# drdh/Homophily-MARL

Measured on AMD Instinct MI355X. Metric: agent_steps_per_sec, higher is better.
Workload: dtype fp32

## Files before the change

### homophily_marl_amd/abi.py

```python
import ctypes as C
import os

ABI_VERSION = 10
MAX_AGENTS = 10
MAX_CELLS = 1024
MAX_SITES = 256

ENV_CLEANUP, ENV_HARVEST = 0, 1
RNG_TAPE, RNG_COUNTER = 0, 1
OBS_F32, OBS_BF16, OBS_U8, OBS_CODE = 0, 1, 2, 3
COLOR_SIMPLIFIED, COLOR_FULL = 0, 1
CODE_CLASS, CODE_CHANNEL_MASK = 0, 1
INPUT_LAST_ACTION, INPUT_AGENT_ID, INPUT_REWARD, INPUT_INC_REWARD, INPUT_DISTANCE, INPUT_AGENT_POS = 1, 2, 4, 8, 16, 32
INPUT_OTHERS_LAST_ACTION = 64
INPUT_GATHER_ONEHOT = 0x100
PREV_RECORD_BYTES = 16
INPUT_EXPLICIT = 0x80000000
STREAM_UNIFORM, STREAM_MOVE, STREAM_WASTE, STREAM_SPAWN_ROT = 0, 1, 2, 3

SSD_OK, SSD_ERR_INVALID, SSD_ERR_DEVICE, SSD_ERR_NOMEM, SSD_ERR_UNSUPPORTED = 0, -1, -2, -3, -4


class SsdConfig(C.Structure):
    _fields_ = [
# ... 135 lines not shown
                ("recv_inc", C.c_void_p), ("recv_inc_out", C.c_void_p), ("avail_bits", C.c_uint32),
                ("others_rows", C.c_void_p), ("prev_record", C.c_void_p), ("prev_record_out", C.c_void_p), ("onehot_rows", C.c_void_p)]


class SsdPolicyHeadParams(C.Structure):
    _fields_ = [("fc1_w", C.c_void_p), ("fc1_b", C.c_void_p), ("w_i", C.c_void_p * 3), ("w_h", C.c_void_p * 3), ("b_i", C.c_void_p * 3),
                ("b_h", C.c_void_p * 3), ("fc2_w", C.c_void_p), ("fc2_b", C.c_void_p), ("fc2_v_w", C.c_void_p), ("fc2_v_b", C.c_void_p),
                ("n_agents", C.c_int32), ("fc1_in", C.c_int32), ("fc2_in", C.c_int32), ("fc2_out", C.c_int32),
                ("input_flags", C.c_uint32), ("n_actions", C.c_int32), ("others_rows", C.c_void_p), ("onehot_rows", C.c_void_p)]


class SsdPolicyEncodeArgs(C.Structure):
    _fields_ = [("codes", C.c_void_p), ("code_bytes", C.c_int64), ("env_stride", C.c_int64), ("slot_stride", C.c_int64),
                ("agent_stride", C.c_int64), ("slot_t", C.c_void_p),
                ("rows", C.c_int32), ("view_edge", C.c_int32), ("n_agents", C.c_int32), ("agent_major", C.c_int32), ("precision", C.c_int32),
                ("conv_frags", C.c_void_p), ("lin_frags", C.c_void_p), ("conv_b", C.c_void_p), ("lin_b", C.c_void_p),
                ("out", C.c_void_p), ("out_stride", C.c_int32), ("part", C.c_void_p), ("slot_t_copy", C.c_void_p), ("counter_inc", C.c_void_p),
                ("alphabet", C.c_int32), ("act", C.c_void_p), ("slot_add", C.c_int32), ("layout", C.c_int32)]


class SsdTdLossArgs(C.Structure):
    _fields_ = [("batch", C.c_int32), ("t_slots", C.c_int32), ("n_agents", C.c_int32), ("n_actions", C.c_int32), ("sim_horizon", C.c_int32),
                ("double_q", C.c_int32),
                ("gamma_env", C.c_float), ("gamma_inc", C.c_float), ("reward_scale", C.c_float), ("incentive_ratio", C.c_float),
                ("incentive_cost", C.c_float), ("incentive", C.c_float), ("seq_len", C.c_float), ("sim_threshold", C.c_float),
                ("sim_loss_weight", C.c_float),
                ("q_env", C.c_void_p), ("q_inc", C.c_void_p), ("tq_env", C.c_void_p), ("tq_inc", C.c_void_p),
                ("actions", C.c_void_p), ("actions_inc", C.c_void_p), ("avail", C.c_void_p), ("reward", C.c_void_p), ("clean_num", C.c_void_p),
                ("terminated", C.c_void_p), ("filled", C.c_void_p), ("dens", C.c_void_p),
                ("dq_env", C.c_void_p), ("dq_inc", C.c_void_p), ("partials", C.c_void_p), ("consider_others_inc", C.c_int32)]


TD_LOSS_PARTIALS = 16
POLICY_HEAD_FRAGS, POLICY_HEAD_TAIL_FLOATS = 58, 464 + 64


POLICY_TAIL_PIECES = 3


def onehot_rows(n_agents, n_actions, flags):
    return 1 + 2 * n_actions + (n_agents * n_actions if flags & INPUT_OTHERS_LAST_ACTION else 0)


def policy_image_bytes(precision):
    return (56 * precision + 8) * 1024


def policy_tail_piece(precision):
    return 56 * precision + 2 * precision


def policy_frag_piece(precision, F, term):
    if F < 8:
        c, ot = F & 1, F >> 1
    elif F < 56:
        G = (F - 8) % 24
        c, ot = (8 if F >= 32 else 2) + 2 * (G >> 3) + (G & 1), (G & 7) >> 1
    else:
        return 56 * precision + 2 * term + (F - 56)
    return 4 * precision * c + 4 * term + ot


def policy_head_plan(n_env, n_agents, fused_with_encoder=False):
    lib = load_library()
    a, b, c = C.c_int32(0), C.c_int32(0), C.c_int32(0)
    check(lib, lib.ssd_policy_head_plan(n_env, n_agents, int(bool(fused_with_encoder)), C.byref(a), C.byref(b), C.byref(c)))
    return a.value, b.value, c.value


ENCODE_EDGE_MIN, ENCODE_EDGE_MAX, ENCODE_BANDS_MAX = 3, 63, 6


def encode_edge_supported(V):
    return ENCODE_EDGE_MIN <= V <= ENCODE_EDGE_MAX and V % 2 == 1


def encode_band_rows(V):
    O = V - 2
    nb = 1 if O <= 13 else min(ENCODE_BANDS_MAX, (O + 9) // 10)
    return (O + nb - 1) // nb


def encode_bands(V):
    return (V - 2 + encode_band_rows(V) - 1) // encode_band_rows(V)


ENCODE_LAYOUT_TOEPLITZ, ENCODE_LAYOUT_LUT = 0, 1
ENCODE_LUT_TABLE_BYTES = 3 * 64 * 6 * 4


def encode_lut_ksteps(V):
    O, R, nb = V - 2, encode_band_rows(V), encode_bands(V)
    return (nb - 1) * ((R * O + 3) // 4) + ((O - (nb - 1) * R) * O + 3) // 4


def encode_frag_bytes(V, precision, layout=ENCODE_LAYOUT_TOEPLITZ):
    if layout == ENCODE_LAYOUT_LUT:
        return ENCODE_LUT_TABLE_BYTES, encode_lut_ksteps(V) * 2 * precision * 1024
    units = 29 * 2 * 3 if V == 31 else 13 * 3
    return precision * 9 * 1024, units * 2 * precision * 1024


def code_agent_stride(V):
    return (V * V + 15) & ~15


HIP_SIGNATURES["ssd_policy_head_env"] = (C.c_int, [C.POINTER(SsdPolicyHead), C.c_void_p])
HIP_SIGNATURES["ssd_policy_head_inc"] = (C.c_int, [C.POINTER(SsdPolicyHead), C.c_void_p])
HIP_SIGNATURES["ssd_gru_seq_fwd"] = (C.c_int, [C.c_void_p] * 6 + [C.c_int32] * 3 + [C.c_void_p])
HIP_SIGNATURES["ssd_gru_seq_bwd"] = (C.c_int, [C.c_void_p] * 9 + [C.c_int32] * 3 + [C.c_void_p])
# ... 100 lines not shown
```

### homophily_marl_amd/csrc/ssd_policy_mfma.hip

```cpp
#include "ssd_policy_common.h"

namespace ssd {
#define SSD_GLOBAL __attribute__((address_space(1)))


using f32x4 = __attribute__((ext_vector_type(4))) float;
using u32x4 = __attribute__((ext_vector_type(4))) uint32_t;
using u32x2 = __attribute__((ext_vector_type(2))) uint32_t;
using h8 = __attribute__((ext_vector_type(8))) _Float16;
using b8 = __attribute__((ext_vector_type(8))) __bf16;

template <int PREC>
__device__ __forceinline__ f32x4 mma(u32x4 a, u32x4 b, f32x4 c) {
    if constexpr (PREC == 2) return __builtin_amdgcn_mfma_f32_16x16x32_f16(__builtin_bit_cast(h8, a), __builtin_bit_cast(h8, b), c, 0, 0, 0);
    else return __builtin_amdgcn_mfma_f32_16x16x32_bf16(__builtin_bit_cast(b8, a), __builtin_bit_cast(b8, b), c, 0, 0, 0);
}

template <int PREC>
__device__ __forceinline__ void split8(const float (&v)[8], u32x4& hi, u32x4& lo) {
    if constexpr (PREC == 2) {
        h8 h, l;
#pragma unroll
        for (int j = 0; j < 8; ++j) { h[j] = (_Float16)v[j]; l[j] = (_Float16)(v[j] - (float)h[j]); }
        hi = __builtin_bit_cast(u32x4, h); lo = __builtin_bit_cast(u32x4, l);
// ... 34 lines not shown
    for (int p = 0; p < 3; ++p) {
        const f32x2 x = x3[p];
        const f32x2 y = x * c;
        float m0, m1, l0, l1;
        asm("v_max_f32 %0, %1, %2" : "=v"(m0) : "v"(x.x), "v"(y.x));
        asm("v_max_f32 %0, %1, %2" : "=v"(m1) : "v"(x.y), "v"(y.y));
        uint32_t h, l;
        asm("v_cvt_pk_f16_f32 %0, %1, %2" : "=v"(h) : "v"(m0), "v"(m1));
        asm("v_fma_mix_f32 %0, %1, -1.0, %2 op_sel:[0,0,0] op_sel_hi:[1,0,0]" : "=v"(l0) : "v"(h), "v"(m0));
        asm("v_fma_mix_f32 %0, %1, -1.0, %2 op_sel:[1,0,0] op_sel_hi:[1,0,0]" : "=v"(l1) : "v"(h), "v"(m1));
        asm("v_cvt_pk_f16_f32 %0, %1, %2" : "=v"(l) : "v"(l0), "v"(l1));
        hi[p] = h; lo[p] = l;
    }
    hi[3] = 0u; lo[3] = 0u;
#else
    (void)x3; hi = u32x4{0u, 0u, 0u, 0u}; lo = hi;
#endif
}

template <int PREC> __device__ __forceinline__ void store_term(uint8_t* dst, float v, size_t term_stride, int32_t* err) {
    if constexpr (PREC == 2) {
        if (!(fabsf(v) <= F16_MAX) && err) atomicOr(err, ERR_F16_RANGE);
        const _Float16 h = (_Float16)v, l = (_Float16)(v - (float)h);
        *reinterpret_cast<_Float16*>(dst) = h; *reinterpret_cast<_Float16*>(dst + term_stride) = l;
    } else {
        *reinterpret_cast<__bf16*>(dst) = (__bf16)v;
    }
}

#ifdef SSD_STAMPS
static unsigned long long* g_policy_stamps = nullptr;
void set_policy_stamps(unsigned long long* buf) { g_policy_stamps = buf; }
#define PSTAMP_DECL unsigned long long* stamps;
#define PSTAMP_SET(k) (k).stamps = g_policy_stamps
#define PSTAMP_AT(i, v) do { if (a.stamps && lane == 0) a.stamps[((size_t)(blockIdx.y * gridDim.x + blockIdx.x) * (blockDim.x >> 6) + wave) * 16 + (i)] = (v); } while (0)
#define PSTAMP(i) PSTAMP_AT(i, __builtin_amdgcn_s_memtime())
#define PSTAMP_REAL(i) PSTAMP_AT(i, __builtin_amdgcn_s_memrealtime())
#define PSTAMP_DRAINED(i) do { asm volatile("s_waitcnt vmcnt(0) lgkmcnt(0)" ::: "memory"); PSTAMP(i); } while (0)
#else
#define PSTAMP_DECL
#define PSTAMP_SET(k)
#define PSTAMP(i)
#define PSTAMP_REAL(i)
#define PSTAMP_DRAINED(i)
#endif

constexpr float HEAD_WSCALE = 64.f, HEAD_XSCALE = 16.f;
constexpr float ENC_CSCALE = 256.f, ENC_LSCALE = 256.f;

constexpr int HF_WI = 8, HF_WH = 32, HF_FC2 = 56, HF_TOT = SSD_POLICY_HEAD_FRAGS;
constexpr int HT_B1 = 0, HT_BI = 64, HT_BH = 256, HT_B2 = 448, HT_W2O = 464, HT_TOT = SSD_POLICY_HEAD_TAIL_FLOATS;
constexpr int SCRATCH = 16 * 16;
constexpr int HEAD_STEPS = 14;
template <int PREC> constexpr int stream_chunks() { return HEAD_STEPS * 4 * PREC / 8; }
template <int PREC> constexpr int step_piece(int c, int t, int ot) { return 4 * PREC * c + 4 * t + ot; }
template <int PREC> constexpr int res_piece() { return stream_chunks<PREC>() * 8; }
template <int PREC> constexpr int fc2_piece(int t, int s2) { return res_piece<PREC>() + 2 * t + s2; }
template <int PREC> constexpr int tail_piece() { return res_piece<PREC>() + 2 * PREC; }
static_assert(res_piece<2>() + 8 == SSD_POLICY_IMAGE_PIECES(2) && res_piece<1>() + 8 == SSD_POLICY_IMAGE_PIECES(1), "image = stream chunks + resident chunk");
static_assert(tail_piece<2>() + SSD_POLICY_TAIL_PIECES <= SSD_POLICY_IMAGE_PIECES(2) && tail_piece<1>() + SSD_POLICY_TAIL_PIECES <= SSD_POLICY_IMAGE_PIECES(1), "tail fits");
constexpr int cmin(int a, int b) { return a < b ? a : b; }
constexpr int cmax(int a, int b) { return a > b ? a : b; }

__device__ __forceinline__ void dma_piece(const uint8_t* gsrc_lane, uint32_t lds_dst) {
#if defined(__HIP_DEVICE_COMPILE__)
    uint32_t keep;
    asm volatile("s_mov_b32 %0, m0\n\ts_mov_b32 m0, %2\n\ts_nop 0\n\tglobal_load_lds_dwordx4 %1, off\n\ts_mov_b32 m0, %0"
                 : "=&s"(keep) : "v"(gsrc_lane), "s"(lds_dst) : "memory");
#else
    (void)gsrc_lane; (void)lds_dst;
#endif
}
template <int N> __device__ __forceinline__ void wait_vm() {
#if defined(__HIP_DEVICE_COMPILE__)
    asm volatile("s_waitcnt vmcnt(%0)" : : "n"(N) : "memory");
#endif
}
using lds_u32 = __attribute__((address_space(3))) uint32_t;
constexpr int STREAM_AHEAD = 6;
constexpr int head_lds_bytes(int waves, int prec) { return SSD_POLICY_IMAGE_BYTES(prec) + waves * SCRATCH * 4 + 16; }
template <int PREC>
__device__ __forceinline__ void stream_image(const uint8_t* src_lane, uint32_t lds_dst, volatile lds_u32* landed) {
    constexpr int NK = stream_chunks<PREC>(), NC = NK + 1;
    auto issue = [&](int k) {
        const int j = k == 0 ? NK : k - 1;
#pragma unroll
        for (int pc = 0; pc < 8; ++pc) dma_piece(src_lane + (size_t)j * 8192 + pc * 1024, lds_dst + (uint32_t)j * 8192u + (uint32_t)pc * 1024u);
    };
#pragma unroll
    for (int k = 0; k < cmin(STREAM_AHEAD + 1, NC); ++k) issue(k);
#pragma unroll
    for (int k = 0; k < NC; ++k) {
        if (k + STREAM_AHEAD < NC) wait_vm<8 * STREAM_AHEAD>();
        else if (k == NC - 1) wait_vm<0>();
        else if (k == NC - 2) wait_vm<8>();
        else if (k == NC - 3) wait_vm<16>();
        else if (k == NC - 4) wait_vm<24>();
        else if (k == NC - 5) wait_vm<32>();
        else wait_vm<40>();
        *landed = (uint32_t)k;
        if (k + STREAM_AHEAD + 1 < NC) issue(k + STREAM_AHEAD + 1);
    }
}
template <int PREC, int C> __device__ __forceinline__ void chunk_ready(volatile const lds_u32* landed, uint32_t& seen) {
    constexpr int first_piece = step_piece<PREC>(C, 0, 0), j = first_piece >> 3;
    if constexpr ((first_piece & 7) == 0) {
// ... 296 lines not shown
        (void)lane;
        PSTAMP(0);
        PSTAMP_REAL(14);
        if (!LOOP && wave < WAVES) {
            const int bia0 = block - (block / a.bpa) * a.bpa, tile00 = wave * a.bpa + bia0;
            if (tile00 < ((a.N + 15) >> 4)) load_tile_rows<INC, PRE_SMALL>(a, tile00, block / a.bpa, lane, in_rows);
        }
        if (!LOOP) {
            if (!INC) asm volatile("" :: "s"(a.N), "s"(a.n), "s"(a.bpa), "s"(a.h), "s"(a.inputs), "s"(a.weights), "s"(a.eps), "s"(a.step), "s"(a.t_index),
                                         "s"(a.prev_actions), "s"(a.prev_reward), "s"(a.recv), "s"(a.prev_inc), "s"(a.pos), "s"(a.orient), "s"(a.feat_part),
                                         "s"(a.lin_b), "s"(a.feat_bands), "s"(a.avail_bits), "s"(a.pos_scale));
            else asm volatile("" :: "s"(a.N), "s"(a.n), "s"(a.bpa), "s"(a.h), "s"(a.inputs), "s"(a.weights), "s"(a.eps), "s"(a.step), "s"(a.t_index),
                                    "s"(a.actions), "s"(a.pos_pre), "s"(a.orient_pre), "s"(a.reward), "s"(a.clean), "s"(a.den), "s"(a.ep_ret), "s"(a.term),
                                    "s"(a.inp), "s"(a.pos_scale));
        }
        if (wave == WAVES) *landed = 0u;
        __builtin_amdgcn_s_barrier();
        if (wave == WAVES) {
            const int agent = block / a.bpa;
            stream_image<PREC>(a.weights + (size_t)agent * IMAGE_BYTES + lane * 16, (uint32_t)(uintptr_t)lds_raw, landed);
            return;
        }
    }
    auto pass = [&](const HeadK& a, const int lane, const int tile) {
    const int agent = block / a.bpa;
    const int m = lane & 15, q = lane >> 4;
    const int N = a.N, n = a.n;
    const int tiles = (N + 15) >> 4;
    TileIn<INC> in;
    if constexpr (!LOOP) in = in_rows;
    if (!INC) PSTAMP_DRAINED(8);
    if (!INC) PSTAMP(9);
    float eps = *(const float SSD_GLOBAL*)a.eps;
    int64_t step64 = *(const int64_t SSD_GLOBAL*)a.step;
    long slot_t = a.t_index ? (long)*(const int64_t SSD_GLOBAL*)a.t_index : 0;
    if (tile < tiles) {
        if constexpr (LOOP) load_tile<INC, false>(a, tile, agent, lane, in);
        else if (!INC && a.feat_part) { load_tile<INC, false, PRE_SMALL>(a, tile, agent, lane, in); }
        else load_tile<INC, true, PRE_SMALL>(a, tile, agent, lane, in);
    }
    u32x4 prec = {0xFFFFFFFFu, 0xFFFFFFFFu, 0xFFFFFFFFu, 0xFFFFFFFFu};
    if constexpr (GEN >= 2) {
        if (tile < tiles) {
            auto rec = cold_ptr<const uint8_t>(COLD_BASE, gather_slots<INC>() + 8);
            const int b0 = tile * 16 + m, bc0 = b0 < N ? b0 : N - 1;
            prec = *(const u32x4 SSD_GLOBAL*)(rec + (size_t)bc0 * 16);
        }
    }
    f32x4 gsum[4];
    if (!INC) PSTAMP(10);
    uint32_t step = 0;
    bool file = false;
    const uint32_t avail_bits = INC ? 0xFFFFFFFFu : ((a.avail_bits >> 31) ? (a.avail_bits & 0x7FFFFFFFu) : avail_to_bits(a.avail, A));
    if (!INC) PSTAMP_DRAINED(11);
    u32x4 bh[2], bl[2];
    auto range_check = [&](float amax) {
        if (!(amax * XS <= F16_MAX)) {
            auto nerr = COLD(int32_t, numeric_err);
            if (nerr) atomicOr((int32_t*)nerr, ERR_F16_RANGE);
        }
    };
    f32x4 xk[4];
    auto prepare = [&](int tl) {
        const int b = tl * 16 + m;
        const bool valid = b < N;
        const int bc = valid ? b : N - 1;
        f32x4 (&x)[4] = xk;
        if (!INC) {
            x[0] = in.x[0]; x[1] = in.x[1];
            if (a.feat_part) {
#pragma unroll
                for (int ct = 0; ct < 2; ++ct) {
#pragma unroll
                    for (int r = 0; r < 4; ++r) x[ct][r] = leaky(x[ct][r]);
                }
            }
            int o_act = 0, o_id = A, o_r = A + n, o_i = A + n + 1, o_dist = TAIL_ABSENT, o_pos = A + n + 2;
            if (GEN) {
                const uint64_t lay = COLD_U64(tail_layout);
                o_act = (int8_t)lay; o_id = (int8_t)(lay >> 8); o_r = (int8_t)(lay >> 16); o_i = (int8_t)(lay >> 24);
                o_dist = (int8_t)(lay >> 32); o_pos = (int8_t)(lay >> 40);
            }
            const float px = in.p0 / a.pos_scale, py = in.p1 / a.pos_scale;
            int recv = 0;
#pragma unroll
            for (int k = 0; k < 3; ++k) {
                const int g = q + 4 * k;
                const int on = (g < n && g != agent) ? 1 : 0;
                recv += on * ((in.inc[k] == 1) - (in.inc[k] == 2));
            }
            recv += __builtin_popcount(in.rv & 0x01010101u) - __builtin_popcount(in.rv & 0x02020202u);
            recv += __shfl_xor(recv, 16);
            recv += __shfl_xor(recv, 32);
            const float sg_r = (float)((in.pr > 0.f) - (in.pr < 0.f)), sg_i = (float)((recv > 0) - (recv < 0));
            const int c_pa = o_act + in.pa, c_id = o_id + agent;
#pragma unroll
            for (int ct = 2; ct < 4; ++ct) {
#pragma unroll
                for (int r = 0; r < 4; ++r) {
                    const int j = 16 * ct + 4 * q + r - 32;
                    float v = (j == c_pa || j == c_id) ? 1.f : 0.f;
                    v = j == o_r ? sg_r : v;
                    v = j == o_i ? sg_i : v;
                    v = j == o_pos ? px : v;
                    v = j == o_pos + 1 ? py : v;
                    x[ct][r] = v;
                }
// ... 75 lines not shown
#pragma unroll
                        for (int ot = 0; ot < 4; ++ot) part[k][ot] = *(const f32x4 SSD_GLOBAL*)((const uint8_t SSD_GLOBAL*)orows + (size_t)((row * 64u + 16u * ot + 4u * (uint32_t)q) * 4u));
                    }
#pragma unroll
                    for (int k = 0; k < 3; ++k) {
                        if (g0 + k >= SSD_MAX_AGENTS) continue;
#pragma unroll
                        for (int ot = 0; ot < 4; ++ot)
#pragma unroll
                            for (int r = 0; r < 4; ++r) {
                                const float v = part[k][ot][r];
                                gsum[ot][r] += __builtin_bit_cast(float, __builtin_bit_cast(uint32_t, v) & keep[k]);
                            }
                    }
                }
            }
        }
    };
    auto file_inputs = [&](int tl) {
        if (INC) return;
        const int b = tl * 16 + m;
        if (b >= N) return;
        float* in_row = a.inputs + ((size_t)agent * N + b) * 64;
#pragma unroll
        for (int ct = 0; ct < 4; ++ct)
            if (ct >= 2 || a.feat_part) stg128(in_row, (size_t)((16 * ct + 4 * q) * 4), xk[ct]);
        if (q == 0) {
            const size_t er = (size_t)b * n + agent;
            ColdA ca; ColdC cc;
            cold_blocks(COLD_BASE, ca, nullptr, &cc);
            const float o0 = a.orient ? in.o0 : 0.f, o1 = a.orient ? in.o1 : 0.f;
            if (ca.pos_copy) {
                ca.pos_copy[er * 2] = in.p0; ca.pos_copy[er * 2 + 1] = in.p1; ca.orient_copy[er * 2] = o0; ca.orient_copy[er * 2 + 1] = o1;
            }
            if (cc.d_pos && file) {
                const size_t sr = (((size_t)b * a.slots + slot_t) * n + agent) * 2;
                cc.d_pos[sr] = in.p0; cc.d_pos[sr + 1] = in.p1; cc.d_orient[sr] = o0; cc.d_orient[sr + 1] = o1;
            }
        }
    };
    auto hand_counters = [&]() {
      if (block == 0 && tid == 0) {
        if (INC) {
            auto next_t = COLD(int64_t, next_t); auto next_step = COLD(int64_t, next_step);
            if (next_t) *next_t = slot_t + 1;
            if (next_step) *next_step = step64 + 1;
        } else {
            auto t_copy = COLD(int64_t, t_copy); auto step_copy = COLD(int64_t, step_copy);
            if (t_copy) *t_copy = slot_t;
            if (step_copy) *step_copy = step64;
        }
      }
    };
    PSTAMP(12);
    step = (uint32_t)step64;
    file = slot_t < (long)a.slots;
    if (tile < tiles) prepare(tile);
    PSTAMP(13);
    PSTAMP(1);
    const uint8_t* img = lds_raw;
    const float* tail = reinterpret_cast<const float*>(img + (size_t)tail_piece<PREC>() * 1024);
    float* scratch = reinterpret_cast<float*>(lds_raw + IMAGE_BYTES) + wave * SCRATCH;
    auto run_tile = [&]() {
        if (PREC == 2) range_check(amax_tiles<4>(0.f, xk));
        const int b = tile * 16 + m;
        const bool valid = b < N;
        const int bc = valid ? b : N - 1;
        const size_t arow = (size_t)agent * N + bc;
        if (first) PSTAMP(2);
        f32x4 x1[4];
#pragma unroll
        for (int ot = 0; ot < 4; ++ot) x1[ot] = f32x4{0.f, 0.f, 0.f, 0.f};
        Frag4<PREC> fa, fb;
#define SSD_LOAD_STEP(c_, f_) do { chunk_ready<PREC, c_>(landed, seen); frag4_load<PREC>(img, c_, lane, f_); } while (0)
        SSD_LOAD_STEP(0, fa);
        SSD_LOAD_STEP(1, fb);
        frag4_mma<PREC>(fa, bh[0], bl[0], x1);
        SSD_LOAD_STEP(2, fa);
        frag4_mma<PREC>(fb, bh[1], bl[1], x1);
#pragma unroll
        for (int ot = 0; ot < 4; ++ot) {
            const f32x4 bias = *reinterpret_cast<const f32x4*>(tail + HT_B1 + 16 * ot + 4 * q);
#pragma unroll
            for (int r = 0; r < 4; ++r) {
                if constexpr (GEN >= 2) x1[ot][r] = leaky(fmaf(x1[ot][r], INV, bias[r]) + gsum[ot][r]);
                else x1[ot][r] = leaky(fmaf(x1[ot][r], INV, bias[r]));
            }
        }
        if (first) PSTAMP(3);
        float* h_row = a.h + arow * 64;
        f32x4 hp[4];
#pragma unroll
        for (int ct = 0; ct < 4; ++ct) hp[ct] = in.hp[ct];
        f32x4 g[16];
#pragma unroll
        for (int ot = 0; ot < 16; ++ot) g[ot] = f32x4{0.f, 0.f, 0.f, 0.f};
        {
            u32x4 xh[2], xl[2], hh[2], hl[2];
            if (PREC == 2) range_check(amax_tiles<4>(0.f, x1));
            operand<PREC>(x1, XS, xh, xl);
            operand<PREC>(hp, XS, hh, hl);
            SSD_LOAD_STEP(3, fb);   frag4_mma<PREC>(fa, xh[0], xl[0], g);
            SSD_LOAD_STEP(4, fa);   frag4_mma<PREC>(fb, xh[1], xl[1], g);
            SSD_LOAD_STEP(5, fb);   frag4_mma<PREC>(fa, xh[0], xl[0], g + 4);
            SSD_LOAD_STEP(6, fa);   frag4_mma<PREC>(fb, xh[1], xl[1], g + 4);
            SSD_LOAD_STEP(7, fb);   frag4_mma<PREC>(fa, xh[0], xl[0], g + 8);
            SSD_LOAD_STEP(8, fa);   frag4_mma<PREC>(fb, xh[1], xl[1], g + 8);
            SSD_LOAD_STEP(9, fb);   frag4_mma<PREC>(fa, hh[0], hl[0], g);
            SSD_LOAD_STEP(10, fa);  frag4_mma<PREC>(fb, hh[1], hl[1], g);
            SSD_LOAD_STEP(11, fb);  frag4_mma<PREC>(fa, hh[0], hl[0], g + 4);
            SSD_LOAD_STEP(12, fa);  frag4_mma<PREC>(fb, hh[1], hl[1], g + 4);
            SSD_LOAD_STEP(13, fb);  frag4_mma<PREC>(fa, hh[0], hl[0], g + 12);
            frag4_mma<PREC>(fb, hh[1], hl[1], g + 12);
            file_inputs(tile);
            hand_counters();
        }
        if (first) PSTAMP(4);
        u32x4 f2h[2], f2l[2];
#pragma unroll
        for (int s2 = 0; s2 < 2; ++s2) {
            const uint8_t* p2 = img + (size_t)fc2_piece<PREC>(0, s2) * 1024 + lane * 16;
            f2h[s2] = *reinterpret_cast<const u32x4*>(p2);
            if (PREC == 2) f2l[s2] = *reinterpret_cast<const u32x4*>(p2 + 2 * 1024);
        }
        f32x4 hn[4];
#pragma unroll
        for (int ft = 0; ft < 4; ++ft) {
            const f32x4 bir = *reinterpret_cast<const f32x4*>(tail + HT_BI + 16 * ft + 4 * q), bhr = *reinterpret_cast<const f32x4*>(tail + HT_BH + 16 * ft + 4 * q);
            const f32x4 biz = *reinterpret_cast<const f32x4*>(tail + HT_BI + 64 + 16 * ft + 4 * q), bhz = *reinterpret_cast<const f32x4*>(tail + HT_BH + 64 + 16 * ft + 4 * q);
            const f32x4 bin = *reinterpret_cast<const f32x4*>(tail + HT_BI + 128 + 16 * ft + 4 * q), bhn = *reinterpret_cast<const f32x4*>(tail + HT_BH + 128 + 16 * ft + 4 * q);
#pragma unroll
            for (int r = 0; r < 4; ++r) {
                const float rg = sigmoid_fast(fmaf(g[ft][r], INV, bir[r] + bhr[r]));
                const float zg = sigmoid_fast(fmaf(g[4 + ft][r], INV, biz[r] + bhz[r]));
                const float ng = tanh_fast(fmaf(g[8 + ft][r], INV, bin[r]) + rg * fmaf(g[12 + ft][r], INV, bhn[r]));
                hn[ft][r] = (1.f - zg) * ng + zg * hp[ft][r];
            }
            if (valid) stg128(h_row, (size_t)((16 * ft + 4 * q) * 4), hn[ft]);
        }
        if (first) PSTAMP(5);
        f32x4 o2 = f32x4{0.f, 0.f, 0.f, 0.f};
        operand<PREC>(hn, XS, bh, bl);
#pragma unroll
        for (int s2 = 0; s2 < 2; ++s2) {
            if (PREC == 2) { o2 = mma<PREC>(f2l[s2], bh[s2], o2); o2 = mma<PREC>(f2h[s2], bl[s2], o2); }
            o2 = mma<PREC>(f2h[s2], bh[s2], o2);
        }
        {
            const f32x4 b2 = *reinterpret_cast<const f32x4*>(tail + HT_B2 + 4 * q);
#pragma unroll
            for (int r = 0; r < 4; ++r) o2[r] = fmaf(o2[r], INV, b2[r]);
        }
        *reinterpret_cast<f32x4*>(scratch + m * 16 + 4 * q) = o2;
        __builtin_amdgcn_fence(__ATOMIC_ACQ_REL, "wavefront");
        __builtin_amdgcn_wave_barrier();
        if (!INC) {
            const int bb = tile * 16 + lane;
            ColdA ca;
            cold_blocks(COLD_BASE, ca, nullptr, nullptr);
            auto out_actions = ca.out_actions; auto p_act = ca.p_act; auto d_actions = ca.d_actions;
            auto out_i32 = ca.out_actions_i32;
            auto q_out = ca.q_out; auto d_onehot = ca.d_onehot;
            if (lane < 16 && bb < N) {
                float av[16];
#pragma unroll
                for (int k4 = 0; k4 < 4; ++k4) {
// ... 23 lines not shown
            const float* w2o = tail + HT_W2O;
            ColdA ca; ColdB cb;
            cold_blocks(COLD_BASE, ca, &cb, nullptr);
            auto out_actions = ca.out_actions; auto p_inc = cb.p_inc; auto d_actions_inc = cb.d_actions_inc;
            auto q_out = ca.q_out;
            auto recv_out = COLD(uint8_t, recv_out);
            if (first) PSTAMP(9);
            const uint32_t n_magic = (65536u + (uint32_t)n - 1u) / (uint32_t)n;
#pragma unroll
            for (int k = 0; k < 3; ++k) {
                if (first && k == 1) PSTAMP(10);
                if (first && k == 2) PSTAMP(11);
                const int it = lane + 64 * k;
                const int row = (int)(((uint32_t)it * n_magic) >> 16), j = it - row * n, bb = tile * 16 + row;
                if (it >= 16 * n || bb >= N) continue;
                const int aj = in.aj[k];
                float f[7];
                f[0] = in.f[k][0] / a.pos_scale; f[1] = in.f[k][1] / a.pos_scale;
#pragma unroll
                for (int e = 2; e < 7; ++e) f[e] = in.f[k][e];
                const f32x4 sc = *reinterpret_cast<const f32x4*>(scratch + row * 16);
                const f32x4 wa = *reinterpret_cast<const f32x4*>(w2o + aj * 4);
                float av[4];
#pragma unroll
                for (int o = 0; o < 4; ++o) av[o] = sc[o] + wa[o];
#pragma unroll
                for (int e = 0; e < 7; ++e) {
                    const f32x4 we = *reinterpret_cast<const f32x4*>(w2o + (A + e) * 4);
#pragma unroll
                    for (int o = 0; o < 4; ++o) av[o] = fmaf(f[e], we[o], av[o]);
                }
                const uint32_t rq = (uint32_t)((agent * N + bb) * n + j);
                const uint32_t rk = ((a.env_id_base + (uint32_t)bb) * (uint32_t)n + (uint32_t)agent) * (uint32_t)n + (uint32_t)j;
                int act = dueling_pick_bits<3>(av, av[3], 3, 0xFFFFFFFFu, eps, step, a.seed, rk, q_out ? q_out + (size_t)rq * 3 : (decltype(q_out))nullptr);
                if (j == agent) act = 0;
                const size_t pair = ((size_t)bb * n + agent) * n + j;
                out_actions[pair] = act;
                if (p_inc) p_inc[pair] = act;
                if (recv_out) recv_out[((size_t)j * N + bb) * 16 + agent] = (uint8_t)act;
                if (d_actions_inc && file) d_actions_inc[(((size_t)bb * a.slots + slot_t) * n + agent) * n + j] = act;
            }
            const int br = tile * 16 + lane;
            if (lane < 16 && br < N && cb.d_reward) {
                const size_t ea = (size_t)br * n + agent, sr = ((size_t)br * a.slots + slot_t) * n + agent;
                if (file) { cb.d_reward[sr] = in.own[0]; cb.d_clean[sr] = in.own[1]; cb.d_den[sr] = in.own[2]; }
                if (cb.p_rew) cb.p_rew[ea] = in.own[0];
                if (cb.ep_ret) cb.ep_ret[ea] = in.ep + in.own[0];
                if (agent == 0 && cb.d_term && file) cb.d_term[(size_t)br * a.slots + slot_t] = (uint8_t)in.term;
            }
        }
        __builtin_amdgcn_wave_barrier();
        if (first) PSTAMP(6);
        first = false;
#undef SSD_LOAD_STEP
    };
    if (tile < tiles) run_tile();
    else hand_counters();
    };
    const int lane0 = tid & 63;
    {
        const int bia = block - (block / a_entry.bpa) * a_entry.bpa;
        const int tile0 = wave * a_entry.bpa + bia;
        if constexpr (!LOOP) {
            pass(a_entry, lane0, tile0);
        } else {
            const int stride = a_entry.bpa * WAVES, tiles_all = (a_entry.N + 15) >> 4;
            int tile = tile0;
            do {
                HeadK al;
                refetch_head_args(al, KOFF);
                int lane = lane0;
#if defined(__HIP_DEVICE_COMPILE__)
                asm volatile("" : "+v"(lane));
#endif
                pass(al, lane, tile);
                tile += stride;
#if defined(__HIP_DEVICE_COMPILE__)
                asm volatile("" : "+s"(tile));
#endif
            } while (tile < tiles_all);
        }
    }
    {
        const HeadK& a = a_entry;
        const int lane = lane0;
        (void)a; (void)lane;
        PSTAMP(7);
        PSTAMP_REAL(15);
    }
}

#ifndef SSD_HEAD_WAVES
#define SSD_HEAD_WAVES 8
#endif
constexpr int HEAD_WAVES = SSD_HEAD_WAVES;
#ifndef SSD_HEAD_WAVES_LOOP
#define SSD_HEAD_WAVES_LOOP 8
#endif
constexpr int HEAD_WAVES_LOOP = SSD_HEAD_WAVES_LOOP;
#ifndef SSD_HEAD_WAVES_GATHER
#define SSD_HEAD_WAVES_GATHER 7
#endif
constexpr int HEAD_WAVES_GATHER = SSD_HEAD_WAVES_GATHER;
constexpr int head_waves(bool loop, int gen = 0) { return gen >= 2 ? HEAD_WAVES_GATHER : loop ? HEAD_WAVES_LOOP : HEAD_WAVES; }
constexpr int HEAD_LEAD_BYTES = 2 * 4 + 6 * 8;
template <int INC, int PREC, int AT, int GEN = 0, bool LOOP = false>
__global__ __launch_bounds__((head_waves(LOOP, GEN) + 1) * 64) void k_head(uint32_t p_Nn, int p_bpa, float* p_h, float* p_inputs, const int64_t* p_prev_actions,
                                                                      const float* p_prev_reward, const uint8_t* p_recv, const float* p_pos, HeadK a, HeadCold cold_unused) {
    extern __shared__ __attribute__((aligned(16))) uint8_t lds_raw[];
    if constexpr (LOOP) head_body<INC, PREC, AT, GEN, head_waves(LOOP, GEN), LOOP, HEAD_LEAD_BYTES>(a, lds_raw, (int)blockIdx.x);
// ... 153 lines not shown
    return 32 + ((flags & SSD_INPUT_LAST_ACTION) ? A : 0) + ((flags & SSD_INPUT_AGENT_ID) ? n : 0) + ((flags & SSD_INPUT_REWARD) ? 1 : 0) +
           ((flags & SSD_INPUT_INC_REWARD) ? 1 : 0);
}
__host__ __device__ inline int onehot_dense_row(uint32_t flags, int n, int A, int k) {
    if (k < 32) return k;
    const int start_r = 32 + ((flags & SSD_INPUT_LAST_ACTION) ? A : 0) + ((flags & SSD_INPUT_AGENT_ID) ? n : 0);
    const int start_i = start_r + ((flags & SSD_INPUT_REWARD) ? 1 : 0);
    const int start_d = others_offset(flags, n, A) + ((flags & SSD_INPUT_OTHERS_LAST_ACTION) ? n * A : 0);
    const int start_p = start_d + ((flags & SSD_INPUT_DISTANCE) ? n : 0);
    int j = k - 32;
    if (flags & SSD_INPUT_REWARD) { if (j < 1) return start_r + j; j -= 1; }
    if (flags & SSD_INPUT_INC_REWARD) { if (j < 1) return start_i + j; j -= 1; }
    if (flags & SSD_INPUT_DISTANCE) { if (j < n) return start_d + j; j -= n; }
    if (flags & SSD_INPUT_AGENT_POS) { if (j < 2) return start_p + j; j -= 2; }
    return -1;
}
__host__ __device__ inline int onehot_table_row(uint32_t flags, int n, int A, int agent, int fc1_in, int r) {
    const int full = others_offset(flags, n, A) + ((flags & SSD_INPUT_OTHERS_LAST_ACTION) ? n * A : 0) + ((flags & SSD_INPUT_DISTANCE) ? n : 0) +
                     ((flags & SSD_INPUT_AGENT_POS) ? 2 : 0);
    if (r == 0) return (flags & SSD_INPUT_AGENT_ID) ? 32 + ((flags & SSD_INPUT_LAST_ACTION) ? A : 0) + agent : -1;
    if (r < 1 + A) return (flags & SSD_INPUT_LAST_ACTION) ? 32 + r - 1 : -1;
    if (r < 1 + 2 * A) return fc1_in == full + A ? full + r - 1 - A : -1;
    return others_offset(flags, n, A) + r - 1 - 2 * A;
}
template <int PREC, int MODE>
__device__ __forceinline__ void pack_head_body(const ssd_policy_head_params& p, uint8_t* image, int32_t* err) {
    constexpr bool OTHERS = MODE == 1;
    constexpr size_t IMAGE_BYTES = SSD_POLICY_IMAGE_BYTES(PREC);
    constexpr float WS = PREC == 2 ? HEAD_WSCALE : 1.f;
    const int agent = blockIdx.y, e = blockIdx.x * 256 + threadIdx.x;
    const int blk = OTHERS ? p.n_agents * p.n_actions : 0, off = OTHERS ? others_offset(p.input_flags, p.n_agents, p.n_actions) : 0;
    if (OTHERS && e < blk * 64) p.others_rows[(size_t)agent * blk * 64 + e] = p.fc1_w[((size_t)agent * p.fc1_in + off) * 64 + e];
    if constexpr (MODE == 2) {
        const int rows = SSD_ONEHOT_ROWS(p.n_agents, p.n_actions, p.input_flags);
        if (e < rows * 64) {
            const int src = onehot_table_row(p.input_flags, p.n_agents, p.n_actions, agent, p.fc1_in, e >> 6);
            p.onehot_rows[(size_t)agent * rows * 64 + e] = src >= 0 ? p.fc1_w[((size_t)agent * p.fc1_in + src) * 64 + (e & 63)] : 0.f;
        }
    }
    uint8_t* img = image + (size_t)agent * IMAGE_BYTES;
    if (e < HF_TOT * 512) {
        const int F = e >> 9, lane = (e >> 3) & 63, j = e & 7, q = lane >> 4, m = lane & 15;
        float w = 0.f;
        int piece, term_pieces = 4;
        if (F < HF_WI) {
            const int ot = F >> 1, s = F & 1, out = 16 * ot + m, k = 32 * s + 16 * (j >> 2) + 4 * q + (j & 3);
            if constexpr (MODE == 2) {
                const int row = onehot_dense_row(p.input_flags, p.n_agents, p.n_actions, k);
                if (row >= 0 && row < p.fc1_in) w = p.fc1_w[((size_t)agent * p.fc1_in + row) * 64 + out];
            } else if (OTHERS) {
                const int row = k < off ? k : k + blk;
                if (row < p.fc1_in) w = p.fc1_w[((size_t)agent * p.fc1_in + row) * 64 + out];
            } else if (k < p.fc1_in) w = p.fc1_w[((size_t)agent * p.fc1_in + k) * 64 + out];
            piece = step_piece<PREC>(s, 0, ot);
        } else if (F < HF_FC2) {
            const bool hid = F >= HF_WH;
            const int G = F - (hid ? HF_WH : HF_WI), ot = G >> 1, s = G & 1, out = 16 * ot + m, k = 32 * s + 16 * (j >> 2) + 4 * q + (j & 3);
            const float* W = (hid ? p.w_h : p.w_i)[out >> 6];
            w = W[((size_t)agent * 64 + k) * 64 + (out & 63)];
            piece = step_piece<PREC>((hid ? 8 : 2) + 2 * (ot >> 2) + s, 0, ot & 3);
        } else {
            const int s = F - HF_FC2, k = 32 * s + 16 * (j >> 2) + 4 * q + (j & 3);
            if (m < p.fc2_out) w = p.fc2_w[((size_t)agent * p.fc2_in + k) * p.fc2_out + m];
            else if (m == p.fc2_out) w = p.fc2_v_w[(size_t)agent * p.fc2_in + k];
            piece = fc2_piece<PREC>(0, s); term_pieces = 2;
        }
        store_term<PREC>(img + ((size_t)piece * 64 + lane) * 16 + 2 * j, w * WS, (size_t)term_pieces * 1024, err);
    }
    if (e < HT_TOT) {
        float v = 0.f;
        if (e < HT_BI) v = p.fc1_b[(size_t)agent * 64 + e];
        else if (e < HT_BH) { const int i = e - HT_BI; v = p.b_i[i >> 6][(size_t)agent * 64 + (i & 63)]; }
        else if (e < HT_B2) { const int i = e - HT_BH; v = p.b_h[i >> 6][(size_t)agent * 64 + (i & 63)]; }
        else if (e < HT_W2O) {
            const int o = e - HT_B2;
            if (o < p.fc2_out) v = p.fc2_b[(size_t)agent * p.fc2_out + o]; else if (o == p.fc2_out) v = p.fc2_v_b[agent];
        } else {
            const int i = e - HT_W2O, ee = i >> 2, o = i & 3;
            if (64 + ee < p.fc2_in) {
                if (o < p.fc2_out) v = p.fc2_w[((size_t)agent * p.fc2_in + 64 + ee) * p.fc2_out + o];
                else if (o == p.fc2_out) v = p.fc2_v_w[(size_t)agent * p.fc2_in + 64 + ee];
            }
        }
        reinterpret_cast<float*>(img + (size_t)tail_piece<PREC>() * 1024)[e] = v;
    }
}
template <int PREC>
__global__ __launch_bounds__(256) void k_pack_head(ssd_policy_head_params p, uint8_t* image, int32_t* err) { pack_head_body<PREC, 0>(p, image, err); }
template <int PREC>
__global__ __launch_bounds__(256) void k_pack_head_others(ssd_policy_head_params p, uint8_t* image, int32_t* err) { pack_head_body<PREC, 1>(p, image, err); }
template <int PREC>
__global__ __launch_bounds__(256) void k_pack_head_onehot(ssd_policy_head_params p, uint8_t* image, int32_t* err) { pack_head_body<PREC, 2>(p, image, err); }

void launch_pack_head(const ssd_policy_head_params* p, int prec, void* image, hipStream_t s) {
    const dim3 grid((HF_TOT * 512 + 255) / 256, p->n_agents);
    int32_t* err = numeric_err_word();
    if (p->input_flags & SSD_INPUT_GATHER_ONEHOT) {
        if (prec == 2) hipLaunchKernelGGL(k_pack_head_onehot<2>, grid, dim3(256), 0, s, *p, static_cast<uint8_t*>(image), err);
        else hipLaunchKernelGGL(k_pack_head_onehot<1>, grid, dim3(256), 0, s, *p, static_cast<uint8_t*>(image), err);
    } else if (p->input_flags & SSD_INPUT_OTHERS_LAST_ACTION) {
        if (prec == 2) hipLaunchKernelGGL(k_pack_head_others<2>, grid, dim3(256), 0, s, *p, static_cast<uint8_t*>(image), err);
        else hipLaunchKernelGGL(k_pack_head_others<1>, grid, dim3(256), 0, s, *p, static_cast<uint8_t*>(image), err);
    } else if (prec == 2) hipLaunchKernelGGL(k_pack_head<2>, grid, dim3(256), 0, s, *p, static_cast<uint8_t*>(image), err);
    else hipLaunchKernelGGL(k_pack_head<1>, grid, dim3(256), 0, s, *p, static_cast<uint8_t*>(image), err);
}

template <int V> struct Geo;
template <> struct Geo<15> { static constexpr int O = 13, CP = 16, NXT = 2, XTP = 1, R = 13, NB = 1; };
template <> struct Geo<31> { static constexpr int O = 29, CP = 32, NXT = 4, XTP = 2, R = 10, NB = 3; };
static_assert(Geo<15>::R == SSD_ENCODE_BAND_ROWS(15) && Geo<15>::NB == SSD_ENCODE_BANDS(15) && Geo<31>::R == SSD_ENCODE_BAND_ROWS(31) &&
              Geo<31>::NB == SSD_ENCODE_BANDS(31), "the shipped bands are the header's geometry");
constexpr int ENC_BT_MAX = 5;
#ifndef SSD_ENC_WAVES
// ... 1002 lines not shown
```

Baseline: 340.4 million.

## Reorder policy-head K-steps so hidden-state GRU matmuls run before input prep

Reorders the streamed weight image so the hidden-state (w_h) K-steps come first, followed by fc1 and then the input-gate steps. The hidden-side MFMAs, which depend only on the previous hidden state, are issued before prepare() and fc1 so their work overlaps with input gathering and the streaming of later chunks. How much hidden work is hoisted early depends on the wave count, precision and mode. Weight packing and the Python frag-piece mapping are updated to match the new order. The risk is higher register pressure from keeping the g accumulators and hidden operands live across prepare().

```diff
diff --git a/homophily_marl_amd/abi.py b/homophily_marl_amd/abi.py
--- a/homophily_marl_amd/abi.py
+++ b/homophily_marl_amd/abi.py
@@ -211,10 +211,10 @@
 
 def policy_frag_piece(precision, F, term):
     if F < 8:
-        c, ot = F & 1, F >> 1
+        c, ot = 6 + (F & 1), F >> 1
     elif F < 56:
         G = (F - 8) % 24
-        c, ot = (8 if F >= 32 else 2) + 2 * (G >> 3) + (G & 1), (G & 7) >> 1
+        c, ot = (0 if F >= 32 else 8) + 2 * (G >> 3) + (G & 1), (G & 7) >> 1
     else:
         return 56 * precision + 2 * term + (F - 56)
     return 4 * precision * c + 4 * term + ot
diff --git a/homophily_marl_amd/csrc/ssd_policy_mfma.hip b/homophily_marl_amd/csrc/ssd_policy_mfma.hip
--- a/homophily_marl_amd/csrc/ssd_policy_mfma.hip
+++ b/homophily_marl_amd/csrc/ssd_policy_mfma.hip
@@ -110,6 +110,10 @@
 constexpr int HT_B1 = 0, HT_BI = 64, HT_BH = 256, HT_B2 = 448, HT_W2O = 464, HT_TOT = SSD_POLICY_HEAD_TAIL_FLOATS;
 constexpr int SCRATCH = 16 * 16;
 constexpr int HEAD_STEPS = 14;
+constexpr int hid_step(int g, int s) { return 2 * g + s; }
+constexpr int fc1_step(int s) { return 6 + s; }
+constexpr int in_step(int g, int s) { return 8 + 2 * g + s; }
+static_assert(hid_step(2, 1) + 1 == fc1_step(0) && fc1_step(1) + 1 == in_step(0, 0) && in_step(2, 1) + 1 == HEAD_STEPS, "the chain's K-steps, in order");
 template <int PREC> constexpr int stream_chunks() { return HEAD_STEPS * 4 * PREC / 8; }
 template <int PREC> constexpr int step_piece(int c, int t, int ot) { return 4 * PREC * c + 4 * t + ot; }
 template <int PREC> constexpr int res_piece() { return stream_chunks<PREC>() * 8; }
@@ -512,7 +516,6 @@
     uint32_t step = 0;
     bool file = false;
     const uint32_t avail_bits = INC ? 0xFFFFFFFFu : ((a.avail_bits >> 31) ? (a.avail_bits & 0x7FFFFFFFu) : avail_to_bits(a.avail, A));
-    if (!INC) PSTAMP_DRAINED(11);
     u32x4 bh[2], bl[2];
     auto range_check = [&](float amax) {
         if (!(amax * XS <= F16_MAX)) {
@@ -694,13 +697,37 @@
         }
       }
     };
+    const uint8_t* img = lds_raw;
+    constexpr int HID_EARLY = (PREC == 2 && WAVES + 1 > 8) ? (INC ? (LOOP ? 0 : 2) : 4) : 6;
+    f32x4 g[16];
+    Frag4<PREC> fa, fb;
+    u32x4 hh[2], hl[2];
+#define SSD_LOAD_STEP(c_, f_) do { chunk_ready<PREC, c_>(landed, seen); frag4_load<PREC>(img, c_, lane, f_); } while (0)
+    auto hidden_side = [&]() {
+#pragma unroll
+        for (int ot = 0; ot < 16; ++ot) g[ot] = f32x4{0.f, 0.f, 0.f, 0.f};
+        if constexpr (HID_EARLY > 0) operand<PREC>(in.hp, XS, hh, hl);
+        if (!INC) PSTAMP(9);
+        if constexpr (HID_EARLY == 6) {
+            SSD_LOAD_STEP(hid_step(0, 0), fa);
+            SSD_LOAD_STEP(hid_step(0, 1), fb);  frag4_mma<PREC>(fa, hh[0], hl[0], g);
+            SSD_LOAD_STEP(hid_step(1, 0), fa);  frag4_mma<PREC>(fb, hh[1], hl[1], g);
+            SSD_LOAD_STEP(hid_step(1, 1), fb);  frag4_mma<PREC>(fa, hh[0], hl[0], g + 4);
+            SSD_LOAD_STEP(hid_step(2, 0), fa);  frag4_mma<PREC>(fb, hh[1], hl[1], g + 4);
+            SSD_LOAD_STEP(hid_step(2, 1), fb);  frag4_mma<PREC>(fa, hh[0], hl[0], g + 12);
+            frag4_mma<PREC>(fb, hh[1], hl[1], g + 12);
+        } else if constexpr (HID_EARLY > 0) {
+            SSD_LOAD_STEP(hid_step(0, 0), fa);  frag4_mma<PREC>(fa, hh[0], hl[0], g);
+            SSD_LOAD_STEP(hid_step(0, 1), fa);  frag4_mma<PREC>(fa, hh[1], hl[1], g);
+            if constexpr (HID_EARLY == 4) {
+                SSD_LOAD_STEP(hid_step(1, 0), fa);  frag4_mma<PREC>(fa, hh[0], hl[0], g + 4);
+                SSD_LOAD_STEP(hid_step(1, 1), fa);  frag4_mma<PREC>(fa, hh[1], hl[1], g + 4);
+            }
+        }
+    };
     PSTAMP(12);
     step = (uint32_t)step64;
     file = slot_t < (long)a.slots;
-    if (tile < tiles) prepare(tile);
-    PSTAMP(13);
-    PSTAMP(1);
-    const uint8_t* img = lds_raw;
     const float* tail = reinterpret_cast<const float*>(img + (size_t)tail_piece<PREC>() * 1024);
     float* scratch = reinterpret_cast<float*>(lds_raw + IMAGE_BYTES) + wave * SCRATCH;
     auto run_tile = [&]() {
@@ -713,13 +740,19 @@
         f32x4 x1[4];
 #pragma unroll
         for (int ot = 0; ot < 4; ++ot) x1[ot] = f32x4{0.f, 0.f, 0.f, 0.f};
-        Frag4<PREC> fa, fb;
-#define SSD_LOAD_STEP(c_, f_) do { chunk_ready<PREC, c_>(landed, seen); frag4_load<PREC>(img, c_, lane, f_); } while (0)
-        SSD_LOAD_STEP(0, fa);
-        SSD_LOAD_STEP(1, fb);
-        frag4_mma<PREC>(fa, bh[0], bl[0], x1);
-        SSD_LOAD_STEP(2, fa);
-        frag4_mma<PREC>(fb, bh[1], bl[1], x1);
+        if constexpr (HID_EARLY == 6) {
+            SSD_LOAD_STEP(fc1_step(0), fa);
+            SSD_LOAD_STEP(fc1_step(1), fb);
+            frag4_mma<PREC>(fa, bh[0], bl[0], x1);
+            SSD_LOAD_STEP(in_step(0, 0), fa);
+            frag4_mma<PREC>(fb, bh[1], bl[1], x1);
+        } else {
+            SSD_LOAD_STEP(fc1_step(0), fa);
+            frag4_mma<PREC>(fa, bh[0], bl[0], x1);
+            SSD_LOAD_STEP(fc1_step(1), fb);
+            SSD_LOAD_STEP(in_step(0, 0), fa);
+            frag4_mma<PREC>(fb, bh[1], bl[1], x1);
+        }
 #pragma unroll
         for (int ot = 0; ot < 4; ++ot) {
             const f32x4 bias = *reinterpret_cast<const f32x4*>(tail + HT_B1 + 16 * ot + 4 * q);
@@ -734,26 +767,36 @@
         f32x4 hp[4];
 #pragma unroll
         for (int ct = 0; ct < 4; ++ct) hp[ct] = in.hp[ct];
-        f32x4 g[16];
-#pragma unroll
-        for (int ot = 0; ot < 16; ++ot) g[ot] = f32x4{0.f, 0.f, 0.f, 0.f};
         {
-            u32x4 xh[2], xl[2], hh[2], hl[2];
+            u32x4 xh[2], xl[2];
             if (PREC == 2) range_check(amax_tiles<4>(0.f, x1));
             operand<PREC>(x1, XS, xh, xl);
-            operand<PREC>(hp, XS, hh, hl);
-            SSD_LOAD_STEP(3, fb);   frag4_mma<PREC>(fa, xh[0], xl[0], g);
-            SSD_LOAD_STEP(4, fa);   frag4_mma<PREC>(fb, xh[1], xl[1], g);
-            SSD_LOAD_STEP(5, fb);   frag4_mma<PREC>(fa, xh[0], xl[0], g + 4);
-            SSD_LOAD_STEP(6, fa);   frag4_mma<PREC>(fb, xh[1], xl[1], g + 4);
-            SSD_LOAD_STEP(7, fb);   frag4_mma<PREC>(fa, xh[0], xl[0], g + 8);
-            SSD_LOAD_STEP(8, fa);   frag4_mma<PREC>(fb, xh[1], xl[1], g + 8);
-            SSD_LOAD_STEP(9, fb);   frag4_mma<PREC>(fa, hh[0], hl[0], g);
-            SSD_LOAD_STEP(10, fa);  frag4_mma<PREC>(fb, hh[1], hl[1], g);
-            SSD_LOAD_STEP(11, fb);  frag4_mma<PREC>(fa, hh[0], hl[0], g + 4);
-            SSD_LOAD_STEP(12, fa);  frag4_mma<PREC>(fb, hh[1], hl[1], g + 4);
-            SSD_LOAD_STEP(13, fb);  frag4_mma<PREC>(fa, hh[0], hl[0], g + 12);
-            frag4_mma<PREC>(fb, hh[1], hl[1], g + 12);
+            SSD_LOAD_STEP(in_step(0, 1), fb);   frag4_mma<PREC>(fa, xh[0], xl[0], g);
+            SSD_LOAD_STEP(in_step(1, 0), fa);   frag4_mma<PREC>(fb, xh[1], xl[1], g);
+            SSD_LOAD_STEP(in_step(1, 1), fb);   frag4_mma<PREC>(fa, xh[0], xl[0], g + 4);
+            SSD_LOAD_STEP(in_step(2, 0), fa);   frag4_mma<PREC>(fb, xh[1], xl[1], g + 4);
+            SSD_LOAD_STEP(in_step(2, 1), fb);   frag4_mma<PREC>(fa, xh[0], xl[0], g + 8);
+            if constexpr (HID_EARLY == 6) frag4_mma<PREC>(fb, xh[1], xl[1], g + 8);
+            else if constexpr (HID_EARLY == 0) {
+                operand<PREC>(in.hp, XS, hh, hl);
+                SSD_LOAD_STEP(hid_step(0, 0), fa);  frag4_mma<PREC>(fb, xh[1], xl[1], g + 8);
+                SSD_LOAD_STEP(hid_step(0, 1), fb);  frag4_mma<PREC>(fa, hh[0], hl[0], g);
+                SSD_LOAD_STEP(hid_step(1, 0), fa);  frag4_mma<PREC>(fb, hh[1], hl[1], g);
+                SSD_LOAD_STEP(hid_step(1, 1), fb);  frag4_mma<PREC>(fa, hh[0], hl[0], g + 4);
+                SSD_LOAD_STEP(hid_step(2, 0), fa);  frag4_mma<PREC>(fb, hh[1], hl[1], g + 4);
+                SSD_LOAD_STEP(hid_step(2, 1), fb);  frag4_mma<PREC>(fa, hh[0], hl[0], g + 12);
+                frag4_mma<PREC>(fb, hh[1], hl[1], g + 12);
+            } else if constexpr (HID_EARLY == 2) {
+                SSD_LOAD_STEP(hid_step(1, 0), fa);  frag4_mma<PREC>(fb, xh[1], xl[1], g + 8);
+                SSD_LOAD_STEP(hid_step(1, 1), fb);  frag4_mma<PREC>(fa, hh[0], hl[0], g + 4);
+                SSD_LOAD_STEP(hid_step(2, 0), fa);  frag4_mma<PREC>(fb, hh[1], hl[1], g + 4);
+                SSD_LOAD_STEP(hid_step(2, 1), fb);  frag4_mma<PREC>(fa, hh[0], hl[0], g + 12);
+                frag4_mma<PREC>(fb, hh[1], hl[1], g + 12);
+            } else {
+                SSD_LOAD_STEP(hid_step(2, 0), fa);  frag4_mma<PREC>(fb, xh[1], xl[1], g + 8);
+                SSD_LOAD_STEP(hid_step(2, 1), fb);  frag4_mma<PREC>(fa, hh[0], hl[0], g + 12);
+                frag4_mma<PREC>(fb, hh[1], hl[1], g + 12);
+            }
             file_inputs(tile);
             hand_counters();
         }
@@ -883,10 +926,16 @@
         __builtin_amdgcn_wave_barrier();
         if (first) PSTAMP(6);
         first = false;
+    };
 #undef SSD_LOAD_STEP
-    };
-    if (tile < tiles) run_tile();
-    else hand_counters();
+    if (tile < tiles) {
+        hidden_side();
+        PSTAMP(13);
+        if (!INC) PSTAMP_DRAINED(11);
+        prepare(tile);
+        PSTAMP(1);
+        run_tile();
+    } else hand_counters();
     };
     const int lane0 = tid & 63;
     {
@@ -1146,13 +1195,13 @@
                 const int row = k < off ? k : k + blk;
                 if (row < p.fc1_in) w = p.fc1_w[((size_t)agent * p.fc1_in + row) * 64 + out];
             } else if (k < p.fc1_in) w = p.fc1_w[((size_t)agent * p.fc1_in + k) * 64 + out];
-            piece = step_piece<PREC>(s, 0, ot);
+            piece = step_piece<PREC>(fc1_step(s), 0, ot);
         } else if (F < HF_FC2) {
             const bool hid = F >= HF_WH;
             const int G = F - (hid ? HF_WH : HF_WI), ot = G >> 1, s = G & 1, out = 16 * ot + m, k = 32 * s + 16 * (j >> 2) + 4 * q + (j & 3);
             const float* W = (hid ? p.w_h : p.w_i)[out >> 6];
             w = W[((size_t)agent * 64 + k) * 64 + (out & 63)];
-            piece = step_piece<PREC>((hid ? 8 : 2) + 2 * (ot >> 2) + s, 0, ot & 3);
+            piece = step_piece<PREC>(hid ? hid_step(ot >> 2, s) : in_step(ot >> 2, s), 0, ot & 3);
         } else {
             const int s = F - HF_FC2, k = 32 * s + 16 * (j >> 2) + 4 * q + (j & 3);
             if (m < p.fc2_out) w = p.fc2_w[((size_t)agent * p.fc2_in + k) * p.fc2_out + m];
```

New measurement: 337.6 million. Within noise of the previous version (-0.8%).
